# RKWin93/E2E-MAPPO-for-MT-FJSP

Measured on NVIDIA B200. Metric: MT-FJSP env-steps/sec, higher is better.
Workload: dtype f64

## Files before the change

e2e-mappo-for-mt-fjsp_b200/csrc/mtfjsp_env.cu:

```cuda
#include <cuda_runtime.h>
#include <math.h>
#include <stdint.h>
#include <stdio.h>
#include <stdlib.h>
#include <string.h>

#include <new>
#include <vector>

#include "../../include/mtfjsp.h"

#define MAX_LEAVES 64
#define MAX_PROG 128
#define FULL 0xffffffffu

namespace {

struct Layout {
    int B, J, M, N, E, left_shift;
    int sd_stride, si_stride, xs_stride;
    int o_st, o_ft, o_dur, o_psel, o_scal, o_macc, o_w, o_eacc, o_eleaf, o_ipre, nich, o_sc;
    int o_mach, o_ord, o_rpred, o_cnt, o_misc, o_nxt;
    int o_mind, o_minpt, o_tt;
    int sm_sd, sm_xs, sm_pt, sm_v, sm_leaf, sm_si, sm_off, sm_nxt, sm_tail;
// ... 4 lines not shown
    int nleaves, nprog;
    int leaf_off[MAX_LEAVES];
    int leaf_len[MAX_LEAVES];
    signed char prog[MAX_PROG];
};

struct Params {
    Layout L;
    PwPlan pw;
    double* sd;
    int16_t* si;
    const double* xs;
    const double* t;
    const double* p;
    const double* weights;
    double cfgw[3], divisor, gamma;
    const int32_t* op;
    const int32_t* mach;
    double* reward5;
    double* scaled4;
    uint8_t* done;
    uint8_t* invalid;
    double* info6;
    const int2* act2;
    uint64_t seed, env_offset;
    const int8_t* edge_id;
    int32_t* op_out;
    int32_t* mach_out;
    void* mfea1;
    uint8_t* mmask;
// ... 3 lines not shown
    int rev;
    void* tfea;
    void* mfea;
    float* adj_w;
    int16_t* adj_src;
    uint8_t* jmask;
    int32_t* cand;
    int mask_mode;
    int obs_inc;
    uint8_t* jm_fin;
    uint8_t* jm_esa;
    int32_t* cand_int;
};

enum { MODE_STEP = 1, MODE_OBS = 2, MODE_RESET = 4, MODE_POLICY = 8,
       MODE_HOST = 16 };

#define INFO6_PUT(b_, k_, v_)                                                                               \
    do {                                                                                                    \
        if (P.info6) P.info6[(size_t)(b_) * 6 + (k_)] = (v_);                                               \
        if (P.rec) {                                                                                        \
            unsigned char* r_ = P.rec + (size_t)(b_) * P.rec_stride;                                        \
            if ((k_) == 1) r_[REC_DONE] = (v_) != 0.0 ? 1 : 0;                                              \
            else reinterpret_cast<double*>(r_)[(k_) == 0 ? 0 : (k_) - 1] = (v_);                            \
        }                                                                                                   \
    } while (0)
constexpr int REC_DONE = 40, REC_BITS = 41;
__host__ __device__ constexpr int rec_bytes(int J) { return (REC_BITS + (J + 7) / 8 + J + 7) / 8 * 8; }

__device__ __forceinline__ double warp_max(double v) {
#pragma unroll
// ... 678 lines not shown
    do {                                                                                     \
        if constexpr (REC_STAGED) {                                                          \
            if (P.rec || P.info6) s_pt[(k_)] = (v_);                                         \
            if ((k_) == 1 && P.rec) {   \
                for (int i_ = 0; i_ < RECW - 5; i_++) reinterpret_cast<uint64_t*>(s_pt + 6)[i_] = 0; \
                s_rec[REC_DONE] = (v_) != 0.0 ? 1 : 0;                                       \
            }                                                                                \
        } else {                                                                             \
            INFO6_PUT(b, (k_), (v_));                                                        \
        }                                                                                    \
    } while (0)

    double* g_sd = P.sd + (size_t)bc * S::SD;
    int16_t* g_si = P.si + (size_t)bc * S::SI;
    const double* g_xs = P.xs + (size_t)bc * S::XS;

    int a = 0, m = 0;
    bool sel = false;
    int cj = 0;
    int nsel_step = 0;
    int eid = 0;
    if constexpr ((MODE & MODE_POLICY) != 0) {
        const uint8_t* jsrc = (P.mask_mode == MTFJSP_MASK_ESA ? P.jm_esa : P.jm_fin) + (size_t)bc * J;
        if (gl < J) {
            sel = jsrc[gl] == 0;
            cj = P.cand_int[(size_t)bc * J + gl];
        }
        if (gl < M && P.mfea1 != nullptr) eid = __ldg(P.edge_id + (size_t)bc * M + gl);
        nsel_step = g_si[S::O_MISC + 2];
    } else if (MODE & MODE_STEP) {
        if (P.act2) { const int2 am = __ldg(P.act2 + bc); a = am.x; m = am.y; }
        else { a = __ldg(P.op + bc); m = __ldg(P.mach + bc); }
    }
    uint64_t* s_bar = S::BAR_IN_PAD
                          ? reinterpret_cast<uint64_t*>(smem_raw + (size_t)(warp * EPW) * S::ENV_BYTES + S::RAW)
                          : reinterpret_cast<uint64_t*>(smem_raw + (size_t)S::WARPS * EPW * S::ENV_BYTES) + warp;
    const uint32_t bar = (uint32_t)__cvta_generic_to_shared(s_bar);
    if (lane == 0) {
        asm volatile("mbarrier.init.shared::cta.b64 [%0], 1;" ::"r"(bar));
        asm volatile("fence.mbarrier_init.release.cluster;" ::: "memory");
        asm volatile("mbarrier.arrive.expect_tx.shared::cta.b64 _, [%0], %1;" ::"r"(bar),
                     "r"((uint32_t)(EPW * (S::SM_SD * 8 + S::B_TT + S::SI * 2)))
                     : "memory");
    }
    __syncwarp();
    if (gl == 0) {
        if constexpr (S::COLD) {
            bulk_g2s(s_sd, g_sd, S::HOT * 8, bar);
            bulk_g2s(s_sd + S::HOT, g_sd + 4 * N, S::TAILBLK * 8, bar);
        } else {
            bulk_g2s(s_sd, g_sd, S::SD * 8, bar);
        }
        if constexpr (S::B_TT > 0) bulk_g2s(base + S::B_SD, g_xs + S::O_TT, S::TT * 8, bar);
        bulk_g2s(s_si, g_si, S::SI * 2, bar);
    }
    if constexpr (S::TTG) {
        if (gl < 4) {
            const int o = gl * 16 < M * M - 1 ? gl * 16 : M * M - 1;
            asm volatile("prefetch.global.L1 [%0];" ::"l"(g_xs + S::O_TT + o));
        }
    }
    double tr = 0.0, pr = 0.0;
    int nsel = 1;
    if constexpr ((MODE & MODE_POLICY) != 0) {
        const unsigned jb = (__ballot_sync(FULL, sel) >> (ge * G)) & S::GMASK;
        nsel = __popc(jb);
        const uint64_t genv = P.env_offset + (uint64_t)bc;
        const uint64_t rnd = rand_u64(P.seed, genv, (uint64_t)nsel_step);
        const int kj = (int)(((rnd >> 32) * (uint64_t)nsel) >> 32);
// ... 49 lines not shown
            asm volatile("prefetch.global.L1 [%0];" ::"l"(g_sd + S::O_PSEL + ja * M + gl));
            if (gl == 0 && apos > 0) asm volatile("prefetch.global.L1 [%0];" ::"l"(g_sd + S::O_DUR + ac - 1));
        }
    }
    {
        uint32_t ok;
        do {
            asm volatile(
                "{\n\t.reg .pred p;\n\t"
                "mbarrier.try_wait.parity.shared::cta.b64 p, [%1], 0;\n\t"
                "selp.u32 %0, 1, 0, p;\n\t}"
                : "=r"(ok)
                : "r"(bar)
                : "memory");
        } while (!ok);
    }
    __syncwarp();

    double* __restrict__ s_st = s_sd + S::O_ST;
    double* __restrict__ s_ft = s_sd + S::O_FT;
    double* __restrict__ s_scal = s_sd + S::SM_SCAL;
    double* __restrict__ s_macc = s_sd + S::SM_MACC;
    const double* __restrict__ s_w = s_sd + S::SM_W;
    double* __restrict__ s_sc = s_sd + S::SM_SC;
    auto TT = [&](const int i, const int j) -> double {
        if constexpr (S::NOTT || S::TTG) return __ldg(g_xs + S::O_TT + i * M + j);
        else return s_tt[i * M + j];
    };
    bool stepped = false;
    auto DUR = [&](const int v) -> double {
// ... 377 lines not shown
                if (P.done) P.done[b] = done ? 1 : 0;
                if (P.invalid) P.invalid[b] = 0;
                INFO6_S(0, total); INFO6_S(1, done ? 1.0 : 0.0);
            }
        } else if (active) {
            if (gl < 5 && P.reward5) P.reward5[(size_t)b * 5 + gl] = 0.0;
            if (gl < 4 && P.scaled4) P.scaled4[(size_t)b * 4 + gl] = 0.0;
            if (gl < 6 && gl != 1) INFO6_S(gl, 0.0);
            if (gl == 0) {
                if (P.done) P.done[b] = (s_misc[2] == N) ? 1 : 0;
                if (P.invalid) P.invalid[b] = 1;
                INFO6_S(1, (s_misc[2] == N) ? 1.0 : 0.0);
            }
        }
        __syncwarp();
        if (valid) {
#pragma unroll
            for (int i = gl; i < 20; i += G) {
                if (i < 4) g_sd[S::O_SCAL + i] = s_scal[i];
                else if (i < 7) g_sd[S::O_MACC + mc * 3 + (i - 4)] = s_macc[mc * 3 + (i - 4)];
                else g_sd[S::O_SC + (i - 7)] = s_sc[i - 7];
            }
        }
    }

    {
        const unsigned bal0 = __ballot_sync(FULL, gl < J && nx == 0);
        const unsigned bal1 = __ballot_sync(FULL, gl < J && nx < M);
        const bool first_missing = ((bal0 >> (ge * G)) & S::GMASK) != 0;
        const bool unfinished = ((bal1 >> (ge * G)) & S::GMASK) != 0;
        const double mn = gmin_d<G>(vj);
// ... 132 lines not shown
            if (v >= 0 && v < N && active) emit_row(v, (s_mach[v] >= 0) ? DUR(v) * PSEL(v) : PSEL(v));
        }
        if (inc) {
            if (P.mfea && valid && gl == 0) emit_mach(mc, o_tail);
        } else {
            const int c = (gl < M) ? (int)s_cnt[gl] : 0;
            int incs = c;
#pragma unroll
            for (int o = 1; o < G; o <<= 1) {
                const int n_ = __shfl_up_sync(FULL, incs, o, G);
                if (gl >= o) incs += n_;
            }
            if (P.mfea && gl < M && active) emit_mach(gl, c > 0 ? (int)s_ord[incs - 1] : 0);
        }
    }
}

__global__ void load_kernel(Layout L, const double* __restrict__ t, const double* __restrict__ p,
                            const double* __restrict__ tt, const int32_t* __restrict__ edge, int W, double* xs,
                            int8_t* edge_id) {
    size_t gid = (size_t)blockIdx.x * blockDim.x + threadIdx.x;
    size_t total = (size_t)L.B * L.N;
    if (gid < total) {
        size_t b = gid / L.N;
        int i = (int)(gid % L.N);
        const double* tr = t + gid * L.M;
        const double* pr = p + gid * L.M;
        double mn = INFINITY, mnpt = INFINITY;
        for (int m = 0; m < L.M; m++) {
            double tv = tr[m], ptv = tv * fabs(pr[m]);
// ... 366 lines not shown
    if (total_e1) total_e1[b] = s[1];
}

__global__ void export_scaler_kernel(Layout L, const double* __restrict__ sd, double* R, double* mean, double* S,
                                     int64_t* n) {
    size_t b = (size_t)blockIdx.x * blockDim.x + threadIdx.x;
    if (b >= (size_t)L.B) return;
    const double* s = sd + b * L.sd_stride + L.o_sc;
    for (int k = 0; k < 4; k++) { R[b * 4 + k] = s[k]; mean[b * 4 + k] = s[4 + k]; S[b * 4 + k] = s[8 + k]; }
    n[b] = (int64_t)s[12];
}

__global__ void reset_copy_kernel(Layout L, const double* __restrict__ sd0, const int16_t* __restrict__ si0,
                                  const double* __restrict__ weights, double* __restrict__ sd, int16_t* __restrict__ si,
                                  uint8_t* __restrict__ jm_fin, uint8_t* __restrict__ jm_esa, int32_t* __restrict__ cand) {
    const int wsi = L.si_stride / 4;
    const int per = L.o_sc + wsi + L.J;
    const size_t gid = (size_t)blockIdx.x * blockDim.x + threadIdx.x;
    if (gid >= (size_t)L.B * per) return;
    const size_t b = gid / per;
    const int i = (int)(gid - b * per);
    if (i < L.o_sc) {
        const size_t k = b * L.sd_stride + i;
        sd[k] = (i >= L.o_w && i < L.o_w + 3) ? weights[b * 3 + (i - L.o_w)] : sd0[k];
    } else if (i < L.o_sc + wsi) {
        const size_t k = b * wsi + (i - L.o_sc);
        reinterpret_cast<uint2*>(si)[k] = reinterpret_cast<const uint2*>(si0)[k];
    } else {
        const int j = i - L.o_sc - wsi;
        jm_fin[b * L.J + j] = 0;
        jm_esa[b * L.J + j] = 0;
        cand[b * L.J + j] = j * L.M;
    }
}

thread_local char g_err[512] = "";

int fail(int code, const char* msg, cudaError_t e = cudaSuccess) {
    if (e != cudaSuccess) snprintf(g_err, sizeof g_err, "%s: %s", msg, cudaGetErrorString(e));
    else snprintf(g_err, sizeof g_err, "%s", msg);
    return code;
}

int align_up(int x, int a) { return (x + a - 1) / a * a; }
// ... 12 lines not shown
        pw.prog[pw.nprog++] = -1;
    }
}

}

struct mtfjsp_env {
    Layout L;
    PwPlan pw;
    int device;
    double cfgw[3], divisor, gamma;
    double *sd, *xs, *t, *p;
    double* sd0;
    int16_t* si0;
    bool reset_snap;
    int16_t* si;
    int8_t* edge_id;
    uint8_t *jm_fin, *jm_esa;
    int32_t* cand;
    int32_t *a_op, *a_mach;
    double *r5, *s4, *info6;
    int2* act2;
    unsigned char* rec;
    int rec_stride;
    uint8_t *dn, *inv;
    float* tmp_adj_w;
    int16_t* tmp_adj_src;
    bool loaded, reset_done, force_generic;
    bool obs_inc_enabled, obs_inc_allowed, obs_synced;
    const void* obs_ptrs[4];
// ... 27 lines not shown
    } while (0)

static Params make_params(mtfjsp_env* h) {
    Params P;
    memset(&P, 0, sizeof P);
    P.L = h->L;
    P.pw = h->pw;
    P.sd = h->sd; P.si = h->si; P.xs = h->xs; P.t = h->t; P.p = h->p;
    P.cfgw[0] = h->cfgw[0]; P.cfgw[1] = h->cfgw[1]; P.cfgw[2] = h->cfgw[2];
    P.divisor = h->divisor; P.gamma = h->gamma;
    P.jm_fin = h->jm_fin; P.jm_esa = h->jm_esa; P.cand_int = h->cand;
    P.b0 = 0; P.b1 = h->L.B;
    return P;
}

template <int MODE, typename OutT>
static int launch_env(mtfjsp_env* h, const Params& P, cudaStream_t s) {
    const Layout& L = h->L;
    size_t smem = (size_t)L.smem_per_warp * L.warps_per_block;
    static thread_local int configured_dev = -1;
    static thread_local size_t configured_smem = 0;
    if (configured_dev != h->device || configured_smem < smem) {
        CK(cudaFuncSetAttribute(env_kernel<MODE, OutT>, cudaFuncAttributeMaxDynamicSharedMemorySize, (int)smem),
           "cudaFuncSetAttribute");
        configured_dev = h->device;
        configured_smem = smem;
    }
    int blocks = (P.b1 - P.b0 + L.warps_per_block - 1) / L.warps_per_block;
    env_kernel<MODE, OutT><<<blocks, L.warps_per_block * 32, smem, s>>>(P);
    h->launches++;
    CK(cudaGetLastError(), "env_kernel launch");
    return MTFJSP_OK;
}

template <class S, int MODE, typename OutT>
static int launch_spec(mtfjsp_env* h, const Params& P, cudaStream_t s) {
    const Layout& L = h->L;
    if (L.sd_stride != S::SD || L.si_stride != S::SI || L.xs_stride != S::XS || L.o_sc != S::O_SC || L.o_misc != S::O_MISC ||
        L.o_eacc != S::O_EACC || L.o_eleaf != S::O_ELEAF || L.o_ipre != S::O_IPRE || L.nich != S::NICH || h->pw.nleaves != S::NLEAF)
        return fail(MTFJSP_E_STATE, "specialised kernel layout mismatch");
    static const size_t extra = getenv("MTFJSP_EXTRA_SMEM") ? (size_t)atoi(getenv("MTFJSP_EXTRA_SMEM")) : 0;
    const size_t smem = (size_t)S::WARPS * S::EPW * S::ENV_BYTES + (S::BAR_IN_PAD ? 0 : 16 * ((S::WARPS * 8 + 15) / 16)) + extra;
    static thread_local int configured_dev = -1;
    if (configured_dev != h->device) {
        CK(cudaFuncSetAttribute(env_kernel_s<S, MODE, OutT>, cudaFuncAttributeMaxDynamicSharedMemorySize, (int)smem),
           "cudaFuncSetAttribute");
        configured_dev = h->device;
    }
    const int per_block = S::WARPS * S::EPW;
    const int blocks = (P.b1 - P.b0 + per_block - 1) / per_block;
    Params Q = P;
    if (h->alternate_order && (MODE & MODE_STEP)) {
        Q.rev = h->flip;
        h->flip ^= 1;
    }
// ... 176 lines not shown
    L.sm_tail = off; off += align_up(M, 8) * 2;
    L.smem_per_warp = align_up(off, 16);
    int wpb = 8;
    while (wpb > 1 && (size_t)wpb * L.smem_per_warp > 200 * 1024) wpb >>= 1;
    if ((size_t)wpb * L.smem_per_warp > 227 * 1024) { delete h; return fail(MTFJSP_E_ARG, "instance too large for shared memory"); }
    L.warps_per_block = wpb;
    h->device = device;
    {
        const char* fg = getenv("MTFJSP_FORCE_GENERIC");
        h->force_generic = fg && fg[0] == '1';
        h->host_chunks = getenv("MTFJSP_HOST_CHUNKS") ? atoi(getenv("MTFJSP_HOST_CHUNKS")) : 4;
        h->host_zerocopy = getenv("MTFJSP_HOST_ZEROCOPY") ? atoi(getenv("MTFJSP_HOST_ZEROCOPY")) : (B >= 16384 ? 2 : 1);
        h->fuse_policy = getenv("MTFJSP_FUSE_POLICY") ? atoi(getenv("MTFJSP_FUSE_POLICY")) : 1;
        h->alternate_order = getenv("MTFJSP_ALTERNATE_ORDER") ? atoi(getenv("MTFJSP_ALTERNATE_ORDER")) : 1;
        h->obs_inc_allowed = !(getenv("MTFJSP_OBS_INCREMENTAL") && atoi(getenv("MTFJSP_OBS_INCREMENTAL")) == 0);
    }
    h->cfgw[0] = 0.4; h->cfgw[1] = 0.4; h->cfgw[2] = 0.2; h->divisor = 1.0; h->gamma = 0.99;
    size_t Bs = (size_t)B;
#define ALLOC(ptr, bytes)                                                      \
    do {                                                                       \
        cudaError_t e_ = cudaMalloc((void**)&(ptr), (bytes));                  \
        if (e_ != cudaSuccess) { mtfjsp_destroy(h); return fail(MTFJSP_E_CUDA, "cudaMalloc", e_); } \
        cudaMemset((ptr), 0, (bytes));                                         \
    } while (0)
    ALLOC(h->sd, Bs * L.sd_stride * 8);
    {
        auto up = [](size_t x) { return (x + 255) / 256 * 256; };
        const size_t b_si = up(Bs * L.si_stride * 2), b_jm = up(Bs * J), b_cd = up(Bs * J * 4), b_xs = up(Bs * L.xs_stride * 8);
        h->slab_bytes = b_si + 2 * b_jm + b_cd + b_xs;
        ALLOC(h->slab, h->slab_bytes);
// ... 67 lines not shown
    h->cfgw[0] = w_mk; h->cfgw[1] = w_ec; h->cfgw[2] = w_tt; h->divisor = scaling_divisor; h->gamma = gamma;
    return MTFJSP_OK;
}

int mtfjsp_set_obs_incremental(mtfjsp_env* h, int on) {
    if (!h) return fail(MTFJSP_E_ARG, "null handle");
    h->obs_inc_enabled = on != 0 && h->obs_inc_allowed;
    h->obs_synced = false;
    return MTFJSP_OK;
}

int mtfjsp_load(mtfjsp_env* h, const double* t, const double* p, const double* tt, const int32_t* edge, int W,
                void* stream) {
    if (!h || !t || !p || !tt || !edge || W < 1) return fail(MTFJSP_E_ARG, "mtfjsp_load: bad argument");
    cudaStream_t s = (cudaStream_t)stream;
    CK(cudaSetDevice(h->device), "cudaSetDevice");
    const Layout& L = h->L;
    size_t n = (size_t)L.B * L.N * L.M * 8;
    CK(cudaMemcpyAsync(h->t, t, n, cudaMemcpyDeviceToDevice, s), "copy t");
    CK(cudaMemcpyAsync(h->p, p, n, cudaMemcpyDeviceToDevice, s), "copy p");
    size_t total = (size_t)L.B * (size_t)(L.N > L.M * L.M ? L.N : L.M * L.M);
    load_kernel<<<(unsigned)((total + 255) / 256), 256, 0, s>>>(L, h->t, h->p, tt, edge, W, h->xs, h->edge_id);
    h->launches++;
    CK(cudaGetLastError(), "load_kernel");
    h->loaded = true;
    h->reset_done = false;
    h->obs_synced = false;
    h->reset_snap = false;
    return MTFJSP_OK;
}

int mtfjsp_scaler_init(mtfjsp_env* h, void* stream) {
    if (!h) return fail(MTFJSP_E_ARG, "null handle");
    CK(cudaSetDevice(h->device), "cudaSetDevice");
    size_t n = (size_t)h->L.B * 13;
    scaler_kernel<<<(unsigned)((n + 255) / 256), 256, 0, (cudaStream_t)stream>>>(h->L, h->sd, 1);
    h->launches++;
    CK(cudaGetLastError(), "scaler_kernel");
    return MTFJSP_OK;
}

int mtfjsp_scaler_reset(mtfjsp_env* h, void* stream) {
    if (!h) return fail(MTFJSP_E_ARG, "null handle");
    CK(cudaSetDevice(h->device), "cudaSetDevice");
    size_t n = (size_t)h->L.B * 4;
    scaler_kernel<<<(unsigned)((n + 255) / 256), 256, 0, (cudaStream_t)stream>>>(h->L, h->sd, 0);
    h->launches++;
    CK(cudaGetLastError(), "scaler_kernel");
    return MTFJSP_OK;
}

int mtfjsp_reset(mtfjsp_env* h, const double* weights, void* stream) {
    if (!h || !weights) return fail(MTFJSP_E_ARG, "mtfjsp_reset: bad argument");
    if (!h->loaded) return fail(MTFJSP_E_STATE, "mtfjsp_reset before mtfjsp_load");
    CK(cudaSetDevice(h->device), "cudaSetDevice");
    cudaStream_t s = (cudaStream_t)stream;
    const Layout& L = h->L;
    h->obs_synced = false;
    if (h->reset_snap) {
        const size_t total = (size_t)L.B * (L.o_sc + L.si_stride / 4 + L.J);
        reset_copy_kernel<<<(unsigned)((total + 255) / 256), 256, 0, s>>>(L, h->sd0, h->si0, weights, h->sd, h->si, h->jm_fin,
                                                                      h->jm_esa, h->cand);
        h->launches++;
        CK(cudaGetLastError(), "reset_copy_kernel");
        return MTFJSP_OK;
    }
    Params P = make_params(h);
    P.weights = weights;
    int rc = launch_env<MODE_RESET, double>(h, P, s);
    if (rc != MTFJSP_OK) return rc;
    h->reset_done = true;
    if (!getenv("MTFJSP_RESET_SNAPSHOT") || atoi(getenv("MTFJSP_RESET_SNAPSHOT")) != 0) {
        CK(cudaMemcpyAsync(h->sd0, h->sd, (size_t)L.B * L.sd_stride * 8, cudaMemcpyDeviceToDevice, s), "snapshot sd");
        CK(cudaMemcpyAsync(h->si0, h->si, (size_t)L.B * L.si_stride * 2, cudaMemcpyDeviceToDevice, s), "snapshot si");
        h->reset_snap = true;
    }
    return MTFJSP_OK;
}


int mtfjsp_step(mtfjsp_env* h, const int32_t* op, const int32_t* mach, double* reward5, double* scaled4,
                uint8_t* done, uint8_t* invalid, void* stream) {
    if (!h || !op || !mach) return fail(MTFJSP_E_ARG, "mtfjsp_step: bad argument");
    if (!h->reset_done) return fail(MTFJSP_E_STATE, "mtfjsp_step before mtfjsp_reset");
    CK(cudaSetDevice(h->device), "cudaSetDevice");
    Params P = make_params(h);
    P.op = op; P.mach = mach; P.reward5 = reward5; P.scaled4 = scaled4; P.done = done; P.invalid = invalid;
    h->obs_synced = false;
    return launch_env_auto<MODE_STEP, double>(h, P, (cudaStream_t)stream);
}

int mtfjsp_obs(mtfjsp_env* h, void* task_fea, void* mach_fea, float* adj_w, int16_t* adj_src, uint8_t* job_mask,
               int32_t* candidate, int mask_mode, int dtype, void* stream) {
    if (!h) return fail(MTFJSP_E_ARG, "null handle");
    if (!h->reset_done) return fail(MTFJSP_E_STATE, "mtfjsp_obs before mtfjsp_reset");
    CK(cudaSetDevice(h->device), "cudaSetDevice");
    Params P = make_params(h);
    int rc = fill_obs(h, P, task_fea, mach_fea, adj_w, adj_src, job_mask, candidate, mask_mode, dtype);
    if (rc) return rc;
    rc = dtype == MTFJSP_F64 ? launch_env_auto<MODE_OBS, double>(h, P, (cudaStream_t)stream)
                             : launch_env_auto<MODE_OBS, float>(h, P, (cudaStream_t)stream);
    if (rc == MTFJSP_OK && task_fea && mach_fea && adj_w && !h->obs_synced) obs_mark(h, task_fea, mach_fea, adj_w, adj_src, dtype);
    return rc;
}

int mtfjsp_step_obs(mtfjsp_env* h, const int32_t* op, const int32_t* mach, double* reward5, double* scaled4,
                    uint8_t* done, uint8_t* invalid, void* task_fea, void* mach_fea, float* adj_w, int16_t* adj_src,
                    uint8_t* job_mask, int32_t* candidate, int mask_mode, int dtype, void* stream) {
    if (!h || !op || !mach) return fail(MTFJSP_E_ARG, "mtfjsp_step_obs: bad argument");
    if (!h->reset_done) return fail(MTFJSP_E_STATE, "mtfjsp_step_obs before mtfjsp_reset");
    CK(cudaSetDevice(h->device), "cudaSetDevice");
    const int inc = obs_inc_now(h, task_fea, mach_fea, adj_w, adj_src, dtype);
    int rc = step_obs_range(h, op, mach, reward5, scaled4, done, invalid, nullptr, task_fea, mach_fea, adj_w, adj_src,
                            job_mask, candidate, mask_mode, dtype, 0, h->L.B, (cudaStream_t)stream, nullptr, nullptr, inc);
    if (rc == MTFJSP_OK) obs_mark(h, task_fea, mach_fea, adj_w, adj_src, dtype);
    return rc;
}

int mtfjsp_mfea1(mtfjsp_env* h, const int32_t* op, void* mfea1, uint8_t* mach_mask, int dtype, void* stream) {
    if (!h || !op || !mfea1) return fail(MTFJSP_E_ARG, "mtfjsp_mfea1: bad argument");
    if (!h->reset_done) return fail(MTFJSP_E_STATE, "mtfjsp_mfea1 before mtfjsp_reset");
    CK(cudaSetDevice(h->device), "cudaSetDevice");
    const Layout& L = h->L;
    cudaStream_t s = (cudaStream_t)stream;
    if (dtype != MTFJSP_F32 && dtype != MTFJSP_F64) return fail(MTFJSP_E_ARG, "dtype must be MTFJSP_F32 or MTFJSP_F64");
    {
        int rc = launch_prestep<false>(h, 0, 0, nullptr, const_cast<int32_t*>(op), nullptr, mfea1, mach_mask, dtype, s);
        if (rc != 0) return rc < 0 ? rc : MTFJSP_OK;
    }
    unsigned blocks = (unsigned)((L.B + 127) / 128);
    if (dtype == MTFJSP_F64)
        mfea1_kernel<double><<<blocks, 128, 0, s>>>(L, h->t, h->p, h->xs, h->si, h->edge_id, op, (double*)mfea1, mach_mask);
    else if (dtype == MTFJSP_F32)
        mfea1_kernel<float><<<blocks, 128, 0, s>>>(L, h->t, h->p, h->xs, h->si, h->edge_id, op, (float*)mfea1, mach_mask);
    else
        return fail(MTFJSP_E_ARG, "dtype must be MTFJSP_F32 or MTFJSP_F64");
    h->launches++;
    CK(cudaGetLastError(), "mfea1_kernel");
    return MTFJSP_OK;
}

int mtfjsp_dense_adj(mtfjsp_env* h, void* adj, int dtype, void* stream) {
    if (!h || !adj) return fail(MTFJSP_E_ARG, "mtfjsp_dense_adj: bad argument");
    if (!h->reset_done) return fail(MTFJSP_E_STATE, "mtfjsp_dense_adj before mtfjsp_reset");
    cudaStream_t s = (cudaStream_t)stream;
    int rc = mtfjsp_obs(h, nullptr, nullptr, h->tmp_adj_w, h->tmp_adj_src, nullptr, nullptr, MTFJSP_MASK_ESA, MTFJSP_F32, stream);
    if (rc) return rc;
    if (dtype == MTFJSP_F64) dense_adj_kernel<double><<<h->L.B, 256, 0, s>>>(h->L, h->tmp_adj_w, h->tmp_adj_src, (double*)adj);
    else if (dtype == MTFJSP_F32) dense_adj_kernel<float><<<h->L.B, 256, 0, s>>>(h->L, h->tmp_adj_w, h->tmp_adj_src, (float*)adj);
    else return fail(MTFJSP_E_ARG, "dtype must be MTFJSP_F32 or MTFJSP_F64");
    h->launches++;
    CK(cudaGetLastError(), "dense_adj_kernel");
    return MTFJSP_OK;
}

int mtfjsp_raw_adj(mtfjsp_env* h, int32_t* adj, void* stream) {
    if (!h || !adj) return fail(MTFJSP_E_ARG, "mtfjsp_raw_adj: bad argument");
    if (!h->reset_done) return fail(MTFJSP_E_STATE, "mtfjsp_raw_adj before mtfjsp_reset");
    CK(cudaSetDevice(h->device), "cudaSetDevice");
    cudaStream_t s = (cudaStream_t)stream;
    const Layout& L = h->L;
    CK(cudaMemsetAsync(adj, 0, (size_t)L.B * L.N * L.N * sizeof(int32_t), s), "cudaMemsetAsync");
    const size_t n = (size_t)L.B * L.N;
    raw_adj_kernel<<<(unsigned)((n + 255) / 256), 256, 0, s>>>(L, h->sd, h->si, h->xs, adj);
    h->launches++;
    CK(cudaGetLastError(), "raw_adj_kernel");
    return MTFJSP_OK;
}

int mtfjsp_generate_instances(int B, int J, int M, int E, uint64_t seed, uint64_t env_offset, double* t, double* p, double* tt,
                              int32_t* edge, int W, void* stream) {
    if (B < 1 || J < 1 || M < 2 || M > 64 || E < 1 || E > M || !t || !p || !tt || !edge)
        return fail(MTFJSP_E_ARG, "mtfjsp_generate_instances: bad argument");
    const int avg = M / E, wmin = M - avg * (E - 1);
    if (W < wmin || W < avg || (long long)E * W > (long long)J * M || (long long)M * M > (long long)J * M * 64)
        return fail(MTFJSP_E_ARG, "mtfjsp_generate_instances: edge table width too small (need W >= largest group) or sizes out of range");
    if ((long long)M * M > (long long)J * M) return fail(MTFJSP_E_ARG, "mtfjsp_generate_instances: needs J >= M");
    const size_t n = (size_t)B * J * M;
    instance_gen_kernel<<<(unsigned)((n + 127) / 128), 128, 0, (cudaStream_t)stream>>>(B, J, M, E, W, seed, env_offset, t, p, tt, edge);
    CK(cudaGetLastError(), "instance_gen_kernel");
    return MTFJSP_OK;
}

int mtfjsp_costs(mtfjsp_env* h, double* cost4, double* total_e1, void* stream) {
    if (!h || (!cost4 && !total_e1)) return fail(MTFJSP_E_ARG, "mtfjsp_costs: bad argument");
    CK(cudaSetDevice(h->device), "cudaSetDevice");
    costs_kernel<<<(h->L.B + 255) / 256, 256, 0, (cudaStream_t)stream>>>(h->L, h->sd, cost4, total_e1);
    h->launches++;
    CK(cudaGetLastError(), "costs_kernel");
    return MTFJSP_OK;
}

int mtfjsp_export_state(mtfjsp_env* h, int32_t* mach, double* st, double* ft, int32_t* routes, void* stream) {
    if (!h) return fail(MTFJSP_E_ARG, "null handle");
    CK(cudaSetDevice(h->device), "cudaSetDevice");
    cudaStream_t s = (cudaStream_t)stream;
    const Layout& L = h->L;
    if (routes) {
        size_t n = (size_t)L.B * L.M * L.N;
        fill_i32_kernel<<<(unsigned)((n + 255) / 256), 256, 0, s>>>(routes, n, -1);
        h->launches++;
    }
    size_t n = (size_t)L.B * L.N;
    export_kernel<<<(unsigned)((n + 255) / 256), 256, 0, s>>>(L, h->sd, h->si, mach, st, ft, routes);
    h->launches++;
    CK(cudaGetLastError(), "export_kernel");
    return MTFJSP_OK;
}

int mtfjsp_export_scaler(mtfjsp_env* h, double* R, double* mean, double* S, int64_t* n, void* stream) {
    if (!h || !R || !mean || !S || !n) return fail(MTFJSP_E_ARG, "mtfjsp_export_scaler: bad argument");
    CK(cudaSetDevice(h->device), "cudaSetDevice");
    export_scaler_kernel<<<(h->L.B + 255) / 256, 256, 0, (cudaStream_t)stream>>>(h->L, h->sd, R, mean, S, n);
    h->launches++;
    CK(cudaGetLastError(), "export_scaler_kernel");
    return MTFJSP_OK;
}

int mtfjsp_policy_random(mtfjsp_env* h, uint64_t seed, uint64_t env_offset, int mask_mode, int32_t* op,
                         int32_t* mach, void* stream) {
    if (!h || !op || !mach) return fail(MTFJSP_E_ARG, "mtfjsp_policy_random: bad argument");
    if (!h->reset_done) return fail(MTFJSP_E_STATE, "mtfjsp_policy_random before mtfjsp_reset");
    CK(cudaSetDevice(h->device), "cudaSetDevice");
    const uint8_t* jm = mask_mode == MTFJSP_MASK_ESA ? h->jm_esa : h->jm_fin;
    policy_kernel<<<(h->L.B + 127) / 128, 128, 0, (cudaStream_t)stream>>>(h->L, h->t, h->si, jm, h->cand, seed, env_offset, op, mach);
    h->launches++;
    CK(cudaGetLastError(), "policy_kernel");
    return MTFJSP_OK;
}

int mtfjsp_random_step(mtfjsp_env* h, uint64_t seed, uint64_t env_offset, int32_t* op, int32_t* mach, void* mfea1,
                       uint8_t* mach_mask, double* reward5, double* scaled4, uint8_t* done, uint8_t* invalid,
                       void* task_fea, void* mach_fea, float* adj_w, int16_t* adj_src, uint8_t* job_mask,
                       int32_t* candidate, int mask_mode, int dtype, void* stream) {
    if (!h) return fail(MTFJSP_E_ARG, "null handle");
    int32_t* o = op ? op : h->a_op;
    int32_t* mc = mach ? mach : h->a_mach;
    if (!h->reset_done) return fail(MTFJSP_E_STATE, "mtfjsp_random_step before mtfjsp_reset");
    if (dtype != MTFJSP_F32 && dtype != MTFJSP_F64) return fail(MTFJSP_E_ARG, "dtype must be MTFJSP_F32 or MTFJSP_F64");
    CK(cudaSetDevice(h->device), "cudaSetDevice");
    {
        Params P = make_params(h);
        P.reward5 = reward5; P.scaled4 = scaled4; P.done = done; P.invalid = invalid;
        P.seed = seed; P.env_offset = env_offset; P.edge_id = h->edge_id; P.op_out = o; P.mach_out = mc;
        P.mfea1 = mfea1; P.mmask = mach_mask;
        int rf = fill_obs(h, P, task_fea, mach_fea, adj_w, adj_src, job_mask, candidate, mask_mode, dtype);
        if (rf) return rf;
        P.obs_inc = obs_inc_now(h, task_fea, mach_fea, adj_w, adj_src, dtype);
        rf = dtype == MTFJSP_F64 ? launch_random_fused<double>(h, P, (cudaStream_t)stream)
                                 : launch_random_fused<float>(h, P, (cudaStream_t)stream);
        if (rf > 0) obs_mark(h, task_fea, mach_fea, adj_w, adj_src, dtype);
        if (rf != 0) return rf < 0 ? rf : MTFJSP_OK;
    }
    int rc = launch_prestep<true>(h, seed, env_offset, mask_mode == MTFJSP_MASK_ESA ? h->jm_esa : h->jm_fin, o, mc, mfea1,
                                  mach_mask, dtype, (cudaStream_t)stream);
    if (rc < 0) return rc;
    if (rc == 0) {
        rc = mtfjsp_policy_random(h, seed, env_offset, mask_mode, o, mc, stream);
        if (rc) return rc;
        if (mfea1) {
            rc = mtfjsp_mfea1(h, o, mfea1, mach_mask, dtype, stream);
            if (rc) return rc;
        }
    }
    return mtfjsp_step_obs(h, o, mc, reward5, scaled4, done, invalid, task_fea, mach_fea, adj_w, adj_src, job_mask,
                           candidate, mask_mode, dtype, stream);
}

static bool is_pinned(const void* p) {
// ... 200 lines not shown
    }
    CK(cudaGraphLaunch(ent->exec, s), "cudaGraphLaunch");
    h->launches += ent->kernels;
    obs_mark(h, task_fea, mach_fea, adj_w, adj_src, dtype);
    CK(cudaStreamSynchronize(s), "cudaStreamSynchronize");
    return MTFJSP_OK;
}

extern "C" {

int mtfjsp_step_host(mtfjsp_env* h, const int32_t* op_host, const int32_t* mach_host, double* info6_host,
                     uint8_t* job_mask_host, int32_t* candidate_host, void* task_fea, void* mach_fea, float* adj_w,
                     int16_t* adj_src, int mask_mode, int dtype, void* stream) {
    if (!h || !op_host || !mach_host) return fail(MTFJSP_E_ARG, "mtfjsp_step_host: bad argument");
    if (!h->reset_done) return fail(MTFJSP_E_STATE, "mtfjsp_step_host before mtfjsp_reset");
    CK(cudaSetDevice(h->device), "cudaSetDevice");
    HostIO io = {op_host, mach_host, nullptr, info6_host, job_mask_host, candidate_host, nullptr};
    return host_step_impl(h, io, task_fea, mach_fea, adj_w, adj_src, mask_mode, dtype, (cudaStream_t)stream);
}

int mtfjsp_step_host_packed(mtfjsp_env* h, const int32_t* actions_host, void* records_host, void* task_fea, void* mach_fea,
                            float* adj_w, int16_t* adj_src, int mask_mode, int dtype, void* stream) {
    if (!h || !actions_host || !records_host) return fail(MTFJSP_E_ARG, "mtfjsp_step_host_packed: bad argument");
    if (!h->reset_done) return fail(MTFJSP_E_STATE, "mtfjsp_step_host_packed before mtfjsp_reset");
    CK(cudaSetDevice(h->device), "cudaSetDevice");
    HostIO io = {nullptr, nullptr, actions_host, nullptr, nullptr, nullptr, (unsigned char*)records_host};
    return host_step_impl(h, io, task_fea, mach_fea, adj_w, adj_src, mask_mode, dtype, (cudaStream_t)stream);
}

int mtfjsp_host_record_bytes(const mtfjsp_env* h) { return h ? h->rec_stride : 0; }

int64_t mtfjsp_launch_count(const mtfjsp_env* h) { return h ? h->launches : 0; }

int64_t mtfjsp_bytes_per_step(const mtfjsp_env* h, int dtype) {
    if (!h) return 0;
    const int64_t N = h->L.N, M = h->L.M, J = h->L.J;
    int64_t b_state = 18 * N + 42 * M + 8 * J + (N + 7) / 8 + 160;
    int64_t fe = dtype == MTFJSP_F64 ? 8 : 4;
    int64_t b_out = 12 * fe * N + 18 * N + 8 * fe * M + 5 * J + 41;
    return 8 + 2 * b_state + b_out;
// ... 16 lines not shown
```

Measured before the change: 985.7 million.

## Defer reset and fuse snapshot restore into the first step kernel

Reset and scaler-reset no longer launch kernels right away. They record a pending state, and the next step kernel loads its state directly from the reset snapshot, patches in the weights and scaler, and writes the full state back. Any other entry point flushes the pending reset through a reworked per-env reset_copy_kernel, now one block per env with vectorised copies. This removes one or two launches plus a full state round-trip per episode, at the cost of extra host-side pending-state bookkeeping and a full state writeback in the fused path.

After: 1.029 billion (median of 6 runs). 4.4% higher.

```diff
diff --git a/e2e-mappo-for-mt-fjsp_b200/csrc/mtfjsp_env.cu b/e2e-mappo-for-mt-fjsp_b200/csrc/mtfjsp_env.cu
--- a/e2e-mappo-for-mt-fjsp_b200/csrc/mtfjsp_env.cu
+++ b/e2e-mappo-for-mt-fjsp_b200/csrc/mtfjsp_env.cu
@@ -1,3 +1,4 @@
+#include <assert.h>
 #include <cuda_runtime.h>
 #include <math.h>
 #include <stdint.h>
@@ -42,6 +43,9 @@
     const double* t;
     const double* p;
     const double* weights;
+    const double* sd0;
+    const int16_t* si0;
+    int clear_ret;
     double cfgw[3], divisor, gamma;
     const int32_t* op;
     const int32_t* mach;
@@ -75,7 +79,8 @@
 };
 
 enum { MODE_STEP = 1, MODE_OBS = 2, MODE_RESET = 4, MODE_POLICY = 8,
-       MODE_HOST = 16 };
+       MODE_HOST = 16,
+       MODE_FROM_RESET = 32 };
 
 #define INFO6_PUT(b_, k_, v_)                                                                               \
     do {                                                                                                    \
@@ -784,6 +789,13 @@
     double* g_sd = P.sd + (size_t)bc * S::SD;
     int16_t* g_si = P.si + (size_t)bc * S::SI;
     const double* g_xs = P.xs + (size_t)bc * S::XS;
+    constexpr bool fr = (MODE & MODE_FROM_RESET) != 0;
+    static_assert(!fr || (!S::COLD && (MODE & MODE_STEP)), "COLD reads dur / psel from the state record, not the snapshot");
+#ifdef MTFJSP_DEBUG_BOUNDS
+    if (fr) assert(bc < P.L.B && P.L.sd_stride == S::SD && P.L.si_stride == S::SI);
+#endif
+    const double* src_sd = fr ? P.sd0 + (size_t)bc * S::SD : g_sd;
+    const int16_t* src_si = fr ? P.si0 + (size_t)bc * S::SI : g_si;
 
     int a = 0, m = 0;
     bool sel = false;
@@ -793,11 +805,11 @@
     if constexpr ((MODE & MODE_POLICY) != 0) {
         const uint8_t* jsrc = (P.mask_mode == MTFJSP_MASK_ESA ? P.jm_esa : P.jm_fin) + (size_t)bc * J;
         if (gl < J) {
-            sel = jsrc[gl] == 0;
-            cj = P.cand_int[(size_t)bc * J + gl];
+            sel = fr ? true : jsrc[gl] == 0;
+            cj = fr ? gl * M : P.cand_int[(size_t)bc * J + gl];
         }
         if (gl < M && P.mfea1 != nullptr) eid = __ldg(P.edge_id + (size_t)bc * M + gl);
-        nsel_step = g_si[S::O_MISC + 2];
+        nsel_step = fr ? 0 : g_si[S::O_MISC + 2];
     } else if (MODE & MODE_STEP) {
         if (P.act2) { const int2 am = __ldg(P.act2 + bc); a = am.x; m = am.y; }
         else { a = __ldg(P.op + bc); m = __ldg(P.mach + bc); }
@@ -810,7 +822,7 @@
         asm volatile("mbarrier.init.shared::cta.b64 [%0], 1;" ::"r"(bar));
         asm volatile("fence.mbarrier_init.release.cluster;" ::: "memory");
         asm volatile("mbarrier.arrive.expect_tx.shared::cta.b64 _, [%0], %1;" ::"r"(bar),
-                     "r"((uint32_t)(EPW * (S::SM_SD * 8 + S::B_TT + S::SI * 2)))
+                     "r"((uint32_t)(EPW * (S::SM_SD * 8 + S::B_TT + S::SI * 2 + (fr ? (S::SD - (S::O_SC & ~1)) * 8 : 0))))
                      : "memory");
     }
     __syncwarp();
@@ -819,10 +831,17 @@
             bulk_g2s(s_sd, g_sd, S::HOT * 8, bar);
             bulk_g2s(s_sd + S::HOT, g_sd + 4 * N, S::TAILBLK * 8, bar);
         } else {
-            bulk_g2s(s_sd, g_sd, S::SD * 8, bar);
+            bulk_g2s(s_sd, src_sd, S::SD * 8, bar);
         }
         if constexpr (S::B_TT > 0) bulk_g2s(base + S::B_SD, g_xs + S::O_TT, S::TT * 8, bar);
-        bulk_g2s(s_si, g_si, S::SI * 2, bar);
+        bulk_g2s(s_si, src_si, S::SI * 2, bar);
+    }
+    constexpr int SC0 = S::O_SC & ~1;
+    static_assert(S::NPT >= S::SD - SC0, "the scaler block is staged in the idle-term scratch");
+    double wv = 0.0;
+    if constexpr (fr) {
+        if (gl == 0) bulk_g2s(s_pt, g_sd + SC0, (S::SD - SC0) * 8, bar);
+        if (gl < 3) wv = P.weights[(size_t)bc * 3 + gl];
     }
     if constexpr (S::TTG) {
         if (gl < 4) {
@@ -902,6 +921,11 @@
                 : "r"(bar)
                 : "memory");
         } while (!ok);
+    }
+    if constexpr (fr) {
+        const double* s_sc0 = s_pt + (S::O_SC - SC0);
+        for (int i = gl; i < 13; i += G) s_sd[S::SM_SC + i] = (i < 4 && P.clear_ret) ? 0.0 : s_sc0[i];
+        if (gl < 3) s_sd[S::SM_W + gl] = wv;
     }
     __syncwarp();
 
@@ -1309,7 +1333,7 @@
             }
         }
         __syncwarp();
-        if (valid) {
+        if (valid && !fr) {
 #pragma unroll
             for (int i = gl; i < 20; i += G) {
                 if (i < 4) g_sd[S::O_SCAL + i] = s_scal[i];
@@ -1472,6 +1496,17 @@
             if (P.mfea && gl < M && active) emit_mach(gl, c > 0 ? (int)s_ord[incs - 1] : 0);
         }
     }
+
+    if (fr && active) {
+        const double2* s2 = reinterpret_cast<const double2*>(s_sd);
+        double2* g2 = reinterpret_cast<double2*>(g_sd);
+#pragma unroll 1
+        for (int i = gl; i < S::SD / 2; i += G) g2[i] = s2[i];
+        const int4* s4 = reinterpret_cast<const int4*>(s_si);
+        int4* g4 = reinterpret_cast<int4*>(g_si);
+#pragma unroll 1
+        for (int i = gl; i < S::SI / 8; i += G) g4[i] = s4[i];
+    }
 }
 
 __global__ void load_kernel(Layout L, const double* __restrict__ t, const double* __restrict__ p,
@@ -1868,20 +1903,19 @@
 __global__ void reset_copy_kernel(Layout L, const double* __restrict__ sd0, const int16_t* __restrict__ si0,
                                   const double* __restrict__ weights, double* __restrict__ sd, int16_t* __restrict__ si,
                                   uint8_t* __restrict__ jm_fin, uint8_t* __restrict__ jm_esa, int32_t* __restrict__ cand) {
-    const int wsi = L.si_stride / 4;
-    const int per = L.o_sc + wsi + L.J;
-    const size_t gid = (size_t)blockIdx.x * blockDim.x + threadIdx.x;
-    if (gid >= (size_t)L.B * per) return;
-    const size_t b = gid / per;
-    const int i = (int)(gid - b * per);
-    if (i < L.o_sc) {
-        const size_t k = b * L.sd_stride + i;
-        sd[k] = (i >= L.o_w && i < L.o_w + 3) ? weights[b * 3 + (i - L.o_w)] : sd0[k];
-    } else if (i < L.o_sc + wsi) {
-        const size_t k = b * wsi + (i - L.o_sc);
-        reinterpret_cast<uint2*>(si)[k] = reinterpret_cast<const uint2*>(si0)[k];
-    } else {
-        const int j = i - L.o_sc - wsi;
+    const size_t b = blockIdx.x;
+    const double2* src = reinterpret_cast<const double2*>(sd0 + b * L.sd_stride);
+    double2* dst = reinterpret_cast<double2*>(sd + b * L.sd_stride);
+    auto word = [&](const int i, const double v) { return (i >= L.o_w && i < L.o_w + 3) ? weights[b * 3 + (i - L.o_w)] : v; };
+    for (int k = threadIdx.x; 2 * k < L.o_sc; k += blockDim.x) {
+        const double2 v = src[k];
+        if (2 * k + 1 < L.o_sc) dst[k] = make_double2(word(2 * k, v.x), word(2 * k + 1, v.y));
+        else sd[b * L.sd_stride + 2 * k] = word(2 * k, v.x);
+    }
+    const int4* si_src = reinterpret_cast<const int4*>(si0 + b * L.si_stride);
+    int4* si_dst = reinterpret_cast<int4*>(si + b * L.si_stride);
+    for (int k = threadIdx.x; k < L.si_stride / 8; k += blockDim.x) si_dst[k] = si_src[k];
+    for (int j = threadIdx.x; j < L.J; j += blockDim.x) {
         jm_fin[b * L.J + j] = 0;
         jm_esa[b * L.J + j] = 0;
         cand[b * L.J + j] = j * L.M;
@@ -1924,6 +1958,9 @@
     double* sd0;
     int16_t* si0;
     bool reset_snap;
+    int fused_reset;
+    bool pend_reset, pend_scaler;
+    const double* pend_w;
     int16_t* si;
     int8_t* edge_id;
     uint8_t *jm_fin, *jm_esa;
@@ -1981,9 +2018,34 @@
     return P;
 }
 
+static int flush_reset(mtfjsp_env* h, cudaStream_t s) {
+    const Layout& L = h->L;
+    if (h->pend_reset) {
+        reset_copy_kernel<<<L.B, 128, 0, s>>>(L, h->sd0, h->si0, h->pend_w, h->sd, h->si, h->jm_fin, h->jm_esa, h->cand);
+        h->launches++;
+        h->pend_reset = false;
+        CK(cudaGetLastError(), "reset_copy_kernel");
+    }
+    if (h->pend_scaler) {
+        const size_t n = (size_t)L.B * 4;
+        scaler_kernel<<<(unsigned)((n + 255) / 256), 256, 0, s>>>(L, h->sd, 0);
+        h->launches++;
+        h->pend_scaler = false;
+        CK(cudaGetLastError(), "scaler_kernel");
+    }
+    return MTFJSP_OK;
+}
+
+static int enter(mtfjsp_env* h, cudaStream_t s, bool step = false) {
+    CK(cudaSetDevice(h->device), "cudaSetDevice");
+    return step ? MTFJSP_OK : flush_reset(h, s);
+}
+
 template <int MODE, typename OutT>
 static int launch_env(mtfjsp_env* h, const Params& P, cudaStream_t s) {
     const Layout& L = h->L;
+    int rc = flush_reset(h, s);
+    if (rc != MTFJSP_OK) return rc;
     size_t smem = (size_t)L.smem_per_warp * L.warps_per_block;
     static thread_local int configured_dev = -1;
     static thread_local size_t configured_smem = 0;
@@ -2006,6 +2068,18 @@
     if (L.sd_stride != S::SD || L.si_stride != S::SI || L.xs_stride != S::XS || L.o_sc != S::O_SC || L.o_misc != S::O_MISC ||
         L.o_eacc != S::O_EACC || L.o_eleaf != S::O_ELEAF || L.o_ipre != S::O_IPRE || L.nich != S::NICH || h->pw.nleaves != S::NLEAF)
         return fail(MTFJSP_E_STATE, "specialised kernel layout mismatch");
+    if constexpr (!S::COLD && (MODE & MODE_STEP) && !(MODE & (MODE_HOST | MODE_FROM_RESET))) {
+        if (h->pend_reset) {
+            Params Q = P;
+            Q.sd0 = h->sd0; Q.si0 = h->si0; Q.weights = h->pend_w; Q.clear_ret = h->pend_scaler ? 1 : 0;
+            h->pend_reset = h->pend_scaler = false;
+            return launch_spec<S, MODE | MODE_FROM_RESET, OutT>(h, Q, s);
+        }
+    }
+    if constexpr (!(MODE & MODE_FROM_RESET)) {
+        const int rc = flush_reset(h, s);
+        if (rc != MTFJSP_OK) return rc;
+    }
     static const size_t extra = getenv("MTFJSP_EXTRA_SMEM") ? (size_t)atoi(getenv("MTFJSP_EXTRA_SMEM")) : 0;
     const size_t smem = (size_t)S::WARPS * S::EPW * S::ENV_BYTES + (S::BAR_IN_PAD ? 0 : 16 * ((S::WARPS * 8 + 15) / 16)) + extra;
     static thread_local int configured_dev = -1;
@@ -2212,6 +2286,7 @@
         h->fuse_policy = getenv("MTFJSP_FUSE_POLICY") ? atoi(getenv("MTFJSP_FUSE_POLICY")) : 1;
         h->alternate_order = getenv("MTFJSP_ALTERNATE_ORDER") ? atoi(getenv("MTFJSP_ALTERNATE_ORDER")) : 1;
         h->obs_inc_allowed = !(getenv("MTFJSP_OBS_INCREMENTAL") && atoi(getenv("MTFJSP_OBS_INCREMENTAL")) == 0);
+        h->fused_reset = getenv("MTFJSP_FUSED_RESET") ? atoi(getenv("MTFJSP_FUSED_RESET")) : 1;
     }
     h->cfgw[0] = 0.4; h->cfgw[1] = 0.4; h->cfgw[2] = 0.2; h->divisor = 1.0; h->gamma = 0.99;
     size_t Bs = (size_t)B;
@@ -2309,7 +2384,8 @@
                 void* stream) {
     if (!h || !t || !p || !tt || !edge || W < 1) return fail(MTFJSP_E_ARG, "mtfjsp_load: bad argument");
     cudaStream_t s = (cudaStream_t)stream;
-    CK(cudaSetDevice(h->device), "cudaSetDevice");
+    int rc = enter(h, s);
+    if (rc) return rc;
     const Layout& L = h->L;
     size_t n = (size_t)L.B * L.N * L.M * 8;
     CK(cudaMemcpyAsync(h->t, t, n, cudaMemcpyDeviceToDevice, s), "copy t");
@@ -2327,7 +2403,8 @@
 
 int mtfjsp_scaler_init(mtfjsp_env* h, void* stream) {
     if (!h) return fail(MTFJSP_E_ARG, "null handle");
-    CK(cudaSetDevice(h->device), "cudaSetDevice");
+    int rc = enter(h, (cudaStream_t)stream);
+    if (rc) return rc;
     size_t n = (size_t)h->L.B * 13;
     scaler_kernel<<<(unsigned)((n + 255) / 256), 256, 0, (cudaStream_t)stream>>>(h->L, h->sd, 1);
     h->launches++;
@@ -2337,7 +2414,12 @@
 
 int mtfjsp_scaler_reset(mtfjsp_env* h, void* stream) {
     if (!h) return fail(MTFJSP_E_ARG, "null handle");
-    CK(cudaSetDevice(h->device), "cudaSetDevice");
+    if (h->pend_reset) {
+        h->pend_scaler = true;
+        return MTFJSP_OK;
+    }
+    int rc = enter(h, (cudaStream_t)stream);
+    if (rc) return rc;
     size_t n = (size_t)h->L.B * 4;
     scaler_kernel<<<(unsigned)((n + 255) / 256), 256, 0, (cudaStream_t)stream>>>(h->L, h->sd, 0);
     h->launches++;
@@ -2348,18 +2430,15 @@
 int mtfjsp_reset(mtfjsp_env* h, const double* weights, void* stream) {
     if (!h || !weights) return fail(MTFJSP_E_ARG, "mtfjsp_reset: bad argument");
     if (!h->loaded) return fail(MTFJSP_E_STATE, "mtfjsp_reset before mtfjsp_load");
-    CK(cudaSetDevice(h->device), "cudaSetDevice");
     cudaStream_t s = (cudaStream_t)stream;
     const Layout& L = h->L;
     h->obs_synced = false;
     if (h->reset_snap) {
-        const size_t total = (size_t)L.B * (L.o_sc + L.si_stride / 4 + L.J);
-        reset_copy_kernel<<<(unsigned)((total + 255) / 256), 256, 0, s>>>(L, h->sd0, h->si0, weights, h->sd, h->si, h->jm_fin,
-                                                                      h->jm_esa, h->cand);
-        h->launches++;
-        CK(cudaGetLastError(), "reset_copy_kernel");
-        return MTFJSP_OK;
-    }
+        h->pend_reset = true;
+        h->pend_w = weights;
+        return h->fused_reset ? MTFJSP_OK : enter(h, s);
+    }
+    CK(cudaSetDevice(h->device), "cudaSetDevice");
     Params P = make_params(h);
     P.weights = weights;
     int rc = launch_env<MODE_RESET, double>(h, P, s);
@@ -2378,7 +2457,8 @@
                 uint8_t* done, uint8_t* invalid, void* stream) {
     if (!h || !op || !mach) return fail(MTFJSP_E_ARG, "mtfjsp_step: bad argument");
     if (!h->reset_done) return fail(MTFJSP_E_STATE, "mtfjsp_step before mtfjsp_reset");
-    CK(cudaSetDevice(h->device), "cudaSetDevice");
+    int rc = enter(h, (cudaStream_t)stream, true);
+    if (rc) return rc;
     Params P = make_params(h);
     P.op = op; P.mach = mach; P.reward5 = reward5; P.scaled4 = scaled4; P.done = done; P.invalid = invalid;
     h->obs_synced = false;
@@ -2389,9 +2469,10 @@
                int32_t* candidate, int mask_mode, int dtype, void* stream) {
     if (!h) return fail(MTFJSP_E_ARG, "null handle");
     if (!h->reset_done) return fail(MTFJSP_E_STATE, "mtfjsp_obs before mtfjsp_reset");
-    CK(cudaSetDevice(h->device), "cudaSetDevice");
+    int rc = enter(h, (cudaStream_t)stream);
+    if (rc) return rc;
     Params P = make_params(h);
-    int rc = fill_obs(h, P, task_fea, mach_fea, adj_w, adj_src, job_mask, candidate, mask_mode, dtype);
+    rc = fill_obs(h, P, task_fea, mach_fea, adj_w, adj_src, job_mask, candidate, mask_mode, dtype);
     if (rc) return rc;
     rc = dtype == MTFJSP_F64 ? launch_env_auto<MODE_OBS, double>(h, P, (cudaStream_t)stream)
                              : launch_env_auto<MODE_OBS, float>(h, P, (cudaStream_t)stream);
@@ -2404,9 +2485,10 @@
                     uint8_t* job_mask, int32_t* candidate, int mask_mode, int dtype, void* stream) {
     if (!h || !op || !mach) return fail(MTFJSP_E_ARG, "mtfjsp_step_obs: bad argument");
     if (!h->reset_done) return fail(MTFJSP_E_STATE, "mtfjsp_step_obs before mtfjsp_reset");
-    CK(cudaSetDevice(h->device), "cudaSetDevice");
+    int rc = enter(h, (cudaStream_t)stream, true);
+    if (rc) return rc;
     const int inc = obs_inc_now(h, task_fea, mach_fea, adj_w, adj_src, dtype);
-    int rc = step_obs_range(h, op, mach, reward5, scaled4, done, invalid, nullptr, task_fea, mach_fea, adj_w, adj_src,
+    rc = step_obs_range(h, op, mach, reward5, scaled4, done, invalid, nullptr, task_fea, mach_fea, adj_w, adj_src,
                             job_mask, candidate, mask_mode, dtype, 0, h->L.B, (cudaStream_t)stream, nullptr, nullptr, inc);
     if (rc == MTFJSP_OK) obs_mark(h, task_fea, mach_fea, adj_w, adj_src, dtype);
     return rc;
@@ -2415,9 +2497,12 @@
 int mtfjsp_mfea1(mtfjsp_env* h, const int32_t* op, void* mfea1, uint8_t* mach_mask, int dtype, void* stream) {
     if (!h || !op || !mfea1) return fail(MTFJSP_E_ARG, "mtfjsp_mfea1: bad argument");
     if (!h->reset_done) return fail(MTFJSP_E_STATE, "mtfjsp_mfea1 before mtfjsp_reset");
-    CK(cudaSetDevice(h->device), "cudaSetDevice");
     const Layout& L = h->L;
     cudaStream_t s = (cudaStream_t)stream;
+    {
+        int rc = enter(h, s);
+        if (rc) return rc;
+    }
     if (dtype != MTFJSP_F32 && dtype != MTFJSP_F64) return fail(MTFJSP_E_ARG, "dtype must be MTFJSP_F32 or MTFJSP_F64");
     {
         int rc = launch_prestep<false>(h, 0, 0, nullptr, const_cast<int32_t*>(op), nullptr, mfea1, mach_mask, dtype, s);
@@ -2439,7 +2524,9 @@
     if (!h || !adj) return fail(MTFJSP_E_ARG, "mtfjsp_dense_adj: bad argument");
     if (!h->reset_done) return fail(MTFJSP_E_STATE, "mtfjsp_dense_adj before mtfjsp_reset");
     cudaStream_t s = (cudaStream_t)stream;
-    int rc = mtfjsp_obs(h, nullptr, nullptr, h->tmp_adj_w, h->tmp_adj_src, nullptr, nullptr, MTFJSP_MASK_ESA, MTFJSP_F32, stream);
+    int rc = enter(h, s);
+    if (rc) return rc;
+    rc = mtfjsp_obs(h, nullptr, nullptr, h->tmp_adj_w, h->tmp_adj_src, nullptr, nullptr, MTFJSP_MASK_ESA, MTFJSP_F32, stream);
     if (rc) return rc;
     if (dtype == MTFJSP_F64) dense_adj_kernel<double><<<h->L.B, 256, 0, s>>>(h->L, h->tmp_adj_w, h->tmp_adj_src, (double*)adj);
     else if (dtype == MTFJSP_F32) dense_adj_kernel<float><<<h->L.B, 256, 0, s>>>(h->L, h->tmp_adj_w, h->tmp_adj_src, (float*)adj);
@@ -2452,8 +2539,9 @@
 int mtfjsp_raw_adj(mtfjsp_env* h, int32_t* adj, void* stream) {
     if (!h || !adj) return fail(MTFJSP_E_ARG, "mtfjsp_raw_adj: bad argument");
     if (!h->reset_done) return fail(MTFJSP_E_STATE, "mtfjsp_raw_adj before mtfjsp_reset");
-    CK(cudaSetDevice(h->device), "cudaSetDevice");
     cudaStream_t s = (cudaStream_t)stream;
+    int rc = enter(h, s);
+    if (rc) return rc;
     const Layout& L = h->L;
     CK(cudaMemsetAsync(adj, 0, (size_t)L.B * L.N * L.N * sizeof(int32_t), s), "cudaMemsetAsync");
     const size_t n = (size_t)L.B * L.N;
@@ -2479,7 +2567,8 @@
 
 int mtfjsp_costs(mtfjsp_env* h, double* cost4, double* total_e1, void* stream) {
     if (!h || (!cost4 && !total_e1)) return fail(MTFJSP_E_ARG, "mtfjsp_costs: bad argument");
-    CK(cudaSetDevice(h->device), "cudaSetDevice");
+    int rc = enter(h, (cudaStream_t)stream);
+    if (rc) return rc;
     costs_kernel<<<(h->L.B + 255) / 256, 256, 0, (cudaStream_t)stream>>>(h->L, h->sd, cost4, total_e1);
     h->launches++;
     CK(cudaGetLastError(), "costs_kernel");
@@ -2488,8 +2577,9 @@
 
 int mtfjsp_export_state(mtfjsp_env* h, int32_t* mach, double* st, double* ft, int32_t* routes, void* stream) {
     if (!h) return fail(MTFJSP_E_ARG, "null handle");
-    CK(cudaSetDevice(h->device), "cudaSetDevice");
     cudaStream_t s = (cudaStream_t)stream;
+    int rc = enter(h, s);
+    if (rc) return rc;
     const Layout& L = h->L;
     if (routes) {
         size_t n = (size_t)L.B * L.M * L.N;
@@ -2505,7 +2595,8 @@
 
 int mtfjsp_export_scaler(mtfjsp_env* h, double* R, double* mean, double* S, int64_t* n, void* stream) {
     if (!h || !R || !mean || !S || !n) return fail(MTFJSP_E_ARG, "mtfjsp_export_scaler: bad argument");
-    CK(cudaSetDevice(h->device), "cudaSetDevice");
+    int rc = enter(h, (cudaStream_t)stream);
+    if (rc) return rc;
     export_scaler_kernel<<<(h->L.B + 255) / 256, 256, 0, (cudaStream_t)stream>>>(h->L, h->sd, R, mean, S, n);
     h->launches++;
     CK(cudaGetLastError(), "export_scaler_kernel");
@@ -2516,7 +2607,8 @@
                          int32_t* mach, void* stream) {
     if (!h || !op || !mach) return fail(MTFJSP_E_ARG, "mtfjsp_policy_random: bad argument");
     if (!h->reset_done) return fail(MTFJSP_E_STATE, "mtfjsp_policy_random before mtfjsp_reset");
-    CK(cudaSetDevice(h->device), "cudaSetDevice");
+    int rc = enter(h, (cudaStream_t)stream);
+    if (rc) return rc;
     const uint8_t* jm = mask_mode == MTFJSP_MASK_ESA ? h->jm_esa : h->jm_fin;
     policy_kernel<<<(h->L.B + 127) / 128, 128, 0, (cudaStream_t)stream>>>(h->L, h->t, h->si, jm, h->cand, seed, env_offset, op, mach);
     h->launches++;
@@ -2533,7 +2625,8 @@
     int32_t* mc = mach ? mach : h->a_mach;
     if (!h->reset_done) return fail(MTFJSP_E_STATE, "mtfjsp_random_step before mtfjsp_reset");
     if (dtype != MTFJSP_F32 && dtype != MTFJSP_F64) return fail(MTFJSP_E_ARG, "dtype must be MTFJSP_F32 or MTFJSP_F64");
-    CK(cudaSetDevice(h->device), "cudaSetDevice");
+    int rc = enter(h, (cudaStream_t)stream, true);
+    if (rc) return rc;
     {
         Params P = make_params(h);
         P.reward5 = reward5; P.scaled4 = scaled4; P.done = done; P.invalid = invalid;
@@ -2547,7 +2640,9 @@
         if (rf > 0) obs_mark(h, task_fea, mach_fea, adj_w, adj_src, dtype);
         if (rf != 0) return rf < 0 ? rf : MTFJSP_OK;
     }
-    int rc = launch_prestep<true>(h, seed, env_offset, mask_mode == MTFJSP_MASK_ESA ? h->jm_esa : h->jm_fin, o, mc, mfea1,
+    rc = flush_reset(h, (cudaStream_t)stream);
+    if (rc) return rc;
+    rc = launch_prestep<true>(h, seed, env_offset, mask_mode == MTFJSP_MASK_ESA ? h->jm_esa : h->jm_fin, o, mc, mfea1,
                                   mach_mask, dtype, (cudaStream_t)stream);
     if (rc < 0) return rc;
     if (rc == 0) {
@@ -2778,7 +2873,8 @@
                      int16_t* adj_src, int mask_mode, int dtype, void* stream) {
     if (!h || !op_host || !mach_host) return fail(MTFJSP_E_ARG, "mtfjsp_step_host: bad argument");
     if (!h->reset_done) return fail(MTFJSP_E_STATE, "mtfjsp_step_host before mtfjsp_reset");
-    CK(cudaSetDevice(h->device), "cudaSetDevice");
+    int rc = enter(h, (cudaStream_t)stream);
+    if (rc) return rc;
     HostIO io = {op_host, mach_host, nullptr, info6_host, job_mask_host, candidate_host, nullptr};
     return host_step_impl(h, io, task_fea, mach_fea, adj_w, adj_src, mask_mode, dtype, (cudaStream_t)stream);
 }
@@ -2787,7 +2883,8 @@
                             float* adj_w, int16_t* adj_src, int mask_mode, int dtype, void* stream) {
     if (!h || !actions_host || !records_host) return fail(MTFJSP_E_ARG, "mtfjsp_step_host_packed: bad argument");
     if (!h->reset_done) return fail(MTFJSP_E_STATE, "mtfjsp_step_host_packed before mtfjsp_reset");
-    CK(cudaSetDevice(h->device), "cudaSetDevice");
+    int rc = enter(h, (cudaStream_t)stream);
+    if (rc) return rc;
     HostIO io = {nullptr, nullptr, actions_host, nullptr, nullptr, nullptr, (unsigned char*)records_host};
     return host_step_impl(h, io, task_fea, mach_fea, adj_w, adj_src, mask_mode, dtype, (cudaStream_t)stream);
 }
diff --git a/profiles/prof_fused_reset.py b/profiles/prof_fused_reset.py
--- /dev/null
+++ b/profiles/prof_fused_reset.py
@@ -0,0 +1,120 @@
+import importlib
+import json
+import os
+import statistics
+import subprocess
+import sys
+
+import torch
+
+ROOT = os.path.dirname(os.path.dirname(os.path.abspath(__file__)))
+sys.path.insert(0, ROOT)
+envm = importlib.import_module("e2e-mappo-for-mt-fjsp_b200.env")
+ins = importlib.import_module("e2e-mappo-for-mt-fjsp_b200.instances")
+
+J, M, E, B, SEED = 6, 6, 2, 65536, 1002
+N = J * M
+K, REPEATS, ROUNDS = 360, 15, int(os.environ.get("ROUNDS", "5"))
+SETTINGS = {"eager_reset": "0", "fused_reset": "1"}
+
+
+def card():
+    try:
+        q = subprocess.run(["nvidia-smi", "--query-gpu=name,power.limit,clocks.max.sm", "--format=csv,noheader"],
+                           capture_output=True, text=True, timeout=30).stdout.strip()
+    except Exception as e:
+        q = "nvidia-smi failed: %r" % e
+    return {"torch_name": torch.cuda.get_device_name(0), "nvidia_smi": q}
+
+
+def make(setting, d, w):
+    os.environ["MTFJSP_FUSED_RESET"] = SETTINGS[setting]
+    env = envm.BatchedMTFJSPEnv(B, J, M, E, left_shift=True, obs_dtype=torch.float32, mask_mode=envm.MASK_ESA)
+    env.load(d["t"], d["p"], d["transT"], d["edge"])
+    env.scaler_init()
+    env.reset(w)
+    return {"env": env, "s": 0}
+
+
+def one_step(st, w):
+    env = st["env"]
+    if st["s"] == N:
+        env.reset(w)
+        env.scaler_reset()
+        st["s"] = 0
+    env.random_step(seed=1234, env_offset=0)
+    st["s"] += 1
+
+
+def timed_region(st, w):
+    times = []
+    for _ in range(REPEATS):
+        e0, e1 = torch.cuda.Event(enable_timing=True), torch.cuda.Event(enable_timing=True)
+        e0.record()
+        for _ in range(K):
+            one_step(st, w)
+        e1.record()
+        torch.cuda.synchronize()
+        times.append(e0.elapsed_time(e1))
+    return statistics.median(times) / K
+
+
+def episode_split(st, w, episodes=3):
+    env = st["env"]
+    steps, heads = [], []
+    for _ in range(episodes):
+        ev = [(torch.cuda.Event(enable_timing=True), torch.cuda.Event(enable_timing=True)) for _ in range(N)]
+        ev[0][0].record()
+        env.reset(w)
+        env.scaler_reset()
+        env.random_step(seed=1234, env_offset=0)
+        ev[0][1].record()
+        for s in range(1, N):
+            ev[s][0].record()
+            env.random_step(seed=1234, env_offset=0)
+            ev[s][1].record()
+        torch.cuda.synchronize()
+        steps += [a.elapsed_time(b) for a, b in ev[1:]]
+        heads.append(ev[0][0].elapsed_time(ev[0][1]))
+    st["s"] = N
+    step_us = 1e3 * statistics.mean(steps)
+    return step_us, 1e3 * statistics.median(heads) - step_us
+
+
+def main():
+    torch.cuda.set_device(0)
+    d = ins.synthetic_instances(0, B, J, M, E, SEED)
+    w = torch.as_tensor(ins.random_weights(0, B, SEED)).cuda()
+    envs = {k: make(k, d, w) for k in SETTINGS}
+    for st in envs.values():
+        for _ in range(2 * N):
+            one_step(st, w)
+    rows = []
+    for r in range(ROUNDS):
+        for k, st in envs.items():
+            ms = timed_region(st, w)
+            step_us, reset_us = episode_split(st, w)
+            rows.append({"round": r, "setting": k, "ms_per_step": ms, "step_kernel_us": step_us, "reset_us": reset_us})
+            print("round %d %-14s %.5f ms/step  step kernel %.2f us  reset %.1f us/episode" % (r, k, ms, step_us, reset_us),
+                  flush=True)
+    summary = {}
+    for k in SETTINGS:
+        xs = [x for x in rows if x["setting"] == k]
+        ms = [x["ms_per_step"] for x in xs]
+        summary[k] = {"ms_per_step_median": statistics.median(ms), "ms_per_step_min": min(ms), "ms_per_step_max": max(ms),
+                      "spread": max(ms) - min(ms), "step_kernel_us_median": statistics.median(x["step_kernel_us"] for x in xs),
+                      "reset_us_median": statistics.median(x["reset_us"] for x in xs),
+                      "env_steps_per_s": B / (statistics.median(ms) * 1e-3)}
+    old = summary["eager_reset"]["ms_per_step_median"]
+    for k in SETTINGS:
+        summary[k]["speedup_vs_eager"] = old / summary[k]["ms_per_step_median"]
+    out = {"card": card(), "workload": "J6M6E2 %d envs, K=%d, median of %d regions, %d rounds" % (B, K, REPEATS, ROUNDS),
+           "summary": summary, "rows": rows}
+    print(json.dumps({"card": out["card"], "summary": summary}, indent=1))
+    if len(sys.argv) > 1:
+        with open(sys.argv[1], "w") as f:
+            json.dump(out, f, indent=1)
+
+
+if __name__ == "__main__":
+    main()
```
